# HKUST-Aerial-Robotics/VINS-Mobile

Measured on AMD Instinct MI355X. Metric: VIO frames/sec (KLT+window solve), 640x480/150 feats/W=10, higher is better.
Workload: dtype f64 (solve) / u8+i32+f32 (KLT)

## Files before the change

### include/vio_amd.h

```cpp
#ifndef VIO_AMD_H
#define VIO_AMD_H

#include <stddef.h>
#include <stdint.h>

#ifdef __cplusplus
extern "C" {
#endif

#define VIO_ABI_VERSION 1

#define VIO_OK 0
#define VIO_EINVAL (-1)
#define VIO_ENODEV (-2)
#define VIO_ENOMEM (-3)
#define VIO_ECAP (-4)
#define VIO_ESTATE (-5)
#define VIO_ETIMEOUT (-6)

#define VIO_SIZE_POSE 7
#define VIO_SIZE_SPEEDBIAS 9
#define VIO_MAX_PRIOR_BLOCKS 96

typedef struct VioConfig {
// ... 150 lines not shown
                             int32_t cols, int32_t stride, const double *headers,
                             int32_t publish, VioObs *out_obs ,
                             int32_t *n_obs );

int vio_frontend_submit_images(vio_frontend_t *fe, const uint8_t *gray, int32_t rows,
                               int32_t cols, int32_t stride, int32_t publish);
int vio_frontend_submit_images_async(vio_frontend_t *fe, const uint8_t *gray, int32_t rows, int32_t cols, int32_t stride,
                                     int32_t publish);
int vio_frontend_collect(vio_frontend_t *fe, VioObs *out_obs ,
                         int32_t *n_obs );

int vio_host_register(void *ptr, size_t bytes);
int vio_host_unregister(void *ptr);

int vio_frontend_upload_frames(vio_frontend_t *fe, const uint8_t *gray, int32_t n_frames,
                               int32_t rows, int32_t cols, int32_t stride);
int vio_frontend_step_resident(vio_frontend_t *fe, int32_t frame_index, int32_t publish,
                               void *stream);
int vio_frontend_sync(vio_frontend_t *fe);
int vio_frontend_kernel_ms(vio_frontend_t *fe, double *ms_avg, int32_t *launches);

typedef struct vio_preprocess vio_preprocess_t;
int vio_preprocess_create(int32_t max_frames, int32_t rows, int32_t cols, vio_preprocess_t **out);
void vio_preprocess_destroy(vio_preprocess_t *p);
int vio_preprocess_set_clahe(vio_preprocess_t *p, double clip_limit, int32_t tiles_x, int32_t tiles_y);
int vio_preprocess_run(vio_preprocess_t *p, const uint8_t *pixels, int32_t channels, int32_t n_frames, int32_t stride,
                       uint8_t *gray_out, uint8_t *equalized_out);
int vio_preprocess_run_resident(vio_preprocess_t *p, const void *d_pixels, int32_t channels, int32_t n_frames,
                                int32_t stride, void *d_equalized, void *stream);
int vio_preprocess_sync(vio_preprocess_t *p);
int vio_preprocess_kernel_ms(vio_preprocess_t *p, double *ms_avg, int32_t *launches);

int vio_frontend_get_state(vio_frontend_t *fe, int32_t seq, float *cur_pts ,
                           int32_t *ids, int32_t *track_cnt, int32_t cap, int32_t *n);
int vio_frontend_get_pnp_points(vio_frontend_t *fe, int32_t seq, float *forw_pts , int32_t *ids,
                                int32_t cap, int32_t *n);
int vio_frontend_lk_iterations(vio_frontend_t *fe, int32_t enable, uint64_t *iterations, uint64_t *visits, int32_t levels_cap);

int vio_frontend_set_tracks(vio_frontend_t *fe, int32_t seq, int32_t n, const float *pre_pts,
                            const float *cur_pts, const float *forw_pts, const int32_t *ids,
                            const int32_t *track_cnt, const uint8_t *lk_status);
int vio_frontend_update_tracks(vio_frontend_t *fe, int32_t publish);
int vio_frontend_get_tracks(vio_frontend_t *fe, int32_t seq, float *forw_pts, int32_t *ids,
                            int32_t *track_cnt, int32_t cap, int32_t *n);

int vio_klt_track(const VioConfig *cfg, const uint8_t *prev, const uint8_t *next,
                  int32_t rows, int32_t cols, int32_t stride, const float *prev_pts,
                  int32_t n, float *next_pts, uint8_t *status, float *err);
int vio_good_features(const VioConfig *cfg, const uint8_t *img, const uint8_t *mask,
                      int32_t rows, int32_t cols, int32_t stride, int32_t max_corners,
                      float *corners , int32_t *n_corners);
int vio_fundamental_ransac(const VioConfig *cfg, const float *pts1, const float *pts2,
                           int32_t n, uint8_t *inlier_mask);

typedef struct vio_matcher vio_matcher_t;
int vio_matcher_create(vio_matcher_t **out);
void vio_matcher_destroy(vio_matcher_t *m);
int vio_matcher_search_by_des(vio_matcher_t *m, int32_t n_pairs, const int32_t *n_cur,
                              const int32_t *n_old, const uint64_t *cur_desc,
                              const uint64_t *old_desc, int32_t *best_index,
                              int32_t *best_dist);
int vio_loop_find_connection(vio_matcher_t *m, const VioConfig *cfg, int32_t n_cur,
                             const uint64_t *cur_desc, const float *cur_pts ,
                             int32_t n_old, const uint64_t *old_desc,
                             const float *old_pts ,
                             float *matched_old_pts ,
                             float *matched_old_norm ,
                             uint8_t *status , int32_t *n_inliers);

typedef struct vio_vocabulary vio_vocabulary_t;
int vio_vocabulary_create(const void *blob, size_t bytes, vio_vocabulary_t **out);
int vio_vocabulary_load(const char *path, vio_vocabulary_t **out);
void vio_vocabulary_destroy(vio_vocabulary_t *v);
int vio_vocabulary_info(const vio_vocabulary_t *v, int32_t info[6]);
int vio_vocabulary_get_device(const vio_vocabulary_t *v, int32_t *device);
int vio_vocabulary_transform(vio_vocabulary_t *v, int32_t n_keyframes, const int32_t *n_desc, const uint64_t *desc,
                             int32_t *word_id, double *word_weight, int32_t *bow_count, int32_t *bow_word,
                             double *bow_value, int32_t bow_stride);
typedef struct vio_bow_database vio_bow_database_t;
int vio_bow_database_create(vio_vocabulary_t *v, int32_t max_entries, int32_t max_total_words, vio_bow_database_t **out);
void vio_bow_database_destroy(vio_bow_database_t *d);
int vio_bow_database_size(const vio_bow_database_t *d, int32_t *n_entries);
int vio_bow_database_add(vio_bow_database_t *d, int32_t n, const int32_t *word, const double *value, int32_t *entry_id);
int vio_bow_database_query(vio_bow_database_t *d, int32_t n_queries, const int32_t *bow_count, const int32_t *bow_word,
                           const double *bow_value, int32_t bow_stride, const int32_t *max_id, int32_t max_results,
                           int32_t *n_results, int32_t *entry, double *score, int32_t result_stride);

typedef struct VioLoopDetectorParams {
  int32_t use_nss; float alpha; int32_t k;
  int32_t geom_check;
  int32_t di_levels;
  int32_t dislocal, max_db_results; float min_nss_factor;
  int32_t min_matches_per_group, max_intragroup_gap, max_distance_between_groups, max_distance_between_queries;
  int32_t min_Fpoints; double max_neighbor_ratio;
  double f_threshold, f_confidence; int32_t min_inliers;
} VioLoopDetectorParams;
void vio_loop_detector_params_default(VioLoopDetectorParams *p, float frequency);

enum {
  VIO_LOOP_DETECTED = 0, VIO_LOOP_CLOSE_MATCHES_ONLY = 1, VIO_LOOP_NO_DB_RESULTS = 2, VIO_LOOP_LOW_NSS_FACTOR = 3,
  VIO_LOOP_LOW_SCORES = 4, VIO_LOOP_NO_GROUPS = 5, VIO_LOOP_NO_TEMPORAL_CONSISTENCY = 6,
  VIO_LOOP_NO_GEOMETRICAL_CONSISTENCY = 7
};
typedef struct VioLoopDetection {
  int32_t status;
  int32_t query, match;
// ... 292 lines not shown
```

### vins-mobile_amd/csrc/vio_frontend.hip

```cpp
#include <hip/hip_runtime.h>

#include <type_traits>

#include "vio_exact_math.h"

#include <math.h>
#include <stdint.h>
#include <stdio.h>
#include <string.h>

#include <algorithm>
#include <condition_variable>
#include <memory>
#include <mutex>
#include <thread>
#include <vector>

#include "vio_amd.h"
#include "vio_device.h"
#include "vio_pool.h"

namespace {

constexpr int kMaxLevels = 4;
// ... 132 lines not shown
  }
    VIO_DPPS(0x111, 0xf) VIO_DPPS(0x112, 0xf) VIO_DPPS(0x114, 0xf) VIO_DPPS(0x118, 0xf) VIO_DPPS(0x142, 0xa) VIO_DPPS(0x143, 0xc)
#undef VIO_DPPS
    sp = (float)__builtin_amdgcn_readlane(u[0], 63), sq = (float)__builtin_amdgcn_readlane(u[1], 63);
    return;
  }
  int a = p & 0xffff, b = q & 0xffff, c = p >> 16, d = q >> 16;
#define VIO_DPP4(ctrl, rmask)                                              \
  {                                                                        \
    const int ta = __builtin_amdgcn_update_dpp(0, a, ctrl, rmask, 0xf, false); \
    const int tb = __builtin_amdgcn_update_dpp(0, b, ctrl, rmask, 0xf, false); \
    const int tc = __builtin_amdgcn_update_dpp(0, c, ctrl, rmask, 0xf, false); \
    const int td = __builtin_amdgcn_update_dpp(0, d, ctrl, rmask, 0xf, false); \
    a += ta, b += tb, c += tc, d += td;                                    \
  }
  VIO_DPP4(0x111, 0xf) VIO_DPP4(0x112, 0xf) VIO_DPP4(0x114, 0xf) VIO_DPP4(0x118, 0xf) VIO_DPP4(0x142, 0xa) VIO_DPP4(0x143, 0xc)
#undef VIO_DPP4
  const int sa = __builtin_amdgcn_readlane(a, 63), sb = __builtin_amdgcn_readlane(b, 63), sc = __builtin_amdgcn_readlane(c, 63),
            sd = __builtin_amdgcn_readlane(d, 63);
  sp = (float)sc * 65536.f + (float)sa, sq = (float)sd * 65536.f + (float)sb;
}

__device__ __forceinline__ void wave_sum_exact3(int p, int q, int r, float &sp, float &sq, float &sr) {
  if (wave_all_small(p, q, r)) {
    int w[3] = {p, q, r};
#define VIO_DPPS3(ctrl, rmask)                                                                                       \
  {                                                                                                                   \
    int t[3];                                                                                                         \
    _Pragma("unroll") for (int k = 0; k < 3; k++) t[k] = __builtin_amdgcn_update_dpp(0, w[k], ctrl, rmask, 0xf, false); \
    _Pragma("unroll") for (int k = 0; k < 3; k++) w[k] += t[k];                                                       \
  }
    VIO_DPPS3(0x111, 0xf) VIO_DPPS3(0x112, 0xf) VIO_DPPS3(0x114, 0xf) VIO_DPPS3(0x118, 0xf) VIO_DPPS3(0x142, 0xa) VIO_DPPS3(0x143, 0xc)
#undef VIO_DPPS3
    sp = (float)__builtin_amdgcn_readlane(w[0], 63), sq = (float)__builtin_amdgcn_readlane(w[1], 63), sr = (float)__builtin_amdgcn_readlane(w[2], 63);
    return;
  }
  int u[3] = {p, q, r};
#define VIO_DPPN(N, arr, ctrl, rmask)                                               \
  {                                                                                 \
    int t[N];                                                                       \
    _Pragma("unroll") for (int k = 0; k < N; k++) t[k] = __builtin_amdgcn_update_dpp(0, arr[k], ctrl, rmask, 0xf, false); \
    _Pragma("unroll") for (int k = 0; k < N; k++) arr[k] += t[k];                   \
  }
  VIO_DPPN(3, u, 0x111, 0xf) VIO_DPPN(3, u, 0x112, 0xf) VIO_DPPN(3, u, 0x114, 0xf) VIO_DPPN(3, u, 0x118, 0xf)
  int v[6] = {u[0] & 0xffff, u[1] & 0xffff, u[2] & 0xffff, u[0] >> 16, u[1] >> 16, u[2] >> 16};
  VIO_DPPN(6, v, 0x142, 0xa) VIO_DPPN(6, v, 0x143, 0xc)
#undef VIO_DPPN
  int s[6];
#pragma unroll
  for (int k = 0; k < 6; k++) s[k] = __builtin_amdgcn_readlane(v[k], 63);
  sp = (float)s[3] * 65536.f + (float)s[0], sq = (float)s[4] * 65536.f + (float)s[1], sr = (float)s[5] * 65536.f + (float)s[2];
}

template <bool STATS = false>
__global__ __launch_bounds__(256, 6) void lk_track_kernel(const uint8_t *prev_pyr, const uint8_t *next_pyr, LkParams P,
                                                       const int *n_pts, const float *prev_pts, float *next_pts,
                                                       uint8_t *status, float *err, unsigned long long *stats) {
  __shared__ LkWaveLds lds_all[4];
  const int seq = blockIdx.y;
  const int wave = threadIdx.x >> 6, lane = threadIdx.x & 63;
  const int pt = blockIdx.x * (blockDim.x >> 6) + wave;
  if (pt >= n_pts[seq]) return;
  LkWaveLds &L = lds_all[wave];
  const uint8_t *pp = prev_pyr + (size_t)seq * P.ld.pyr_bytes, *np = next_pyr + (size_t)seq * P.ld.pyr_bytes;
  const size_t pidx = ((size_t)seq * P.cap + pt) * 2;
  const float ptx = prev_pts[pidx], pty = prev_pts[pidx + 1];
  const float half = (kWin - 1) * 0.5f;
  const float FLT_SCALE = 1.f / (1 << 20);
  constexpr int NPX = (kWin * kWin + 63) / 64;
  const int wy0 = min(lane / kWin, 2), wx0 = lane % kWin;
  const int joff = wy0 * kJS + wx0;
  bool st = true;
  float er = 0.f;
  float nxx = 0.f, nxy = 0.f;
  const int max_level = P.ld.levels - 1;
  for (int level = max_level; level >= 0; level--) {
    const int rows = P.ld.rows[level], cols = P.ld.cols[level];
    const uint8_t *I = pp + P.ld.off[level], *J = np + P.ld.off[level];
    if (level == 0) {
      if (P.prev0) I = P.prev0 + (size_t)seq * P.stride0;
      if (P.next0) J = P.next0 + (size_t)seq * P.stride0;
    }
    const float scale = __int_as_float((127 - level) << 23);
    float px = ptx * scale, py = pty * scale;
    float qx, qy;
    if (level == max_level) qx = px, qy = py;
    else qx = nxx * 2.f, qy = nxy * 2.f;
    nxx = qx, nxy = qy;
    px -= half, py -= half;
    int ipx = (int)floorf(px), ipy = (int)floorf(py);
    if (ipx < -kWin || ipx >= cols || ipy < -kWin || ipy >= rows) {
      if (level == 0) st = false, er = 0.f;
      continue;
    }
    float a = px - ipx, b = py - ipy;
    int iw00, iw01, iw10, iw11;
    lk_weights(a, b, iw00, iw01, iw10, iw11);
    wave_lds_fence();
    if (ipx >= 1 && ipx + kIP - 1 <= cols && ipy >= 1 && ipy + kIP - 1 <= rows) {
      const int r = lane / 6, d = lane - 6 * r;
      constexpr int TI = (kIP + 9) / 10;
      uint32_t curs[TI];
#pragma unroll
      for (int t = 0; t < TI; t++) {
        const int ly = r + 10 * t;
        curs[t] = lk_load4(I + (unsigned)(__mul24(ipy - 1 + (ly < kIP ? ly : 0), cols) + ipx - 1 + 4 * d));
      }
// ... 168 lines not shown
      __builtin_memcpy(&bot, &b32, 4);
      return __builtin_amdgcn_sdot2(bot, wbot, (int)__builtin_amdgcn_udot2(top, wtop, (unsigned)Ic[q], false), false) >> (kWBits - 5);
    };
    int nit = 0;
    for (int j = 0; j < P.max_count; j++) {
      int iqx = (int)floorf(qx), iqy = (int)floorf(qy);
      if (iqx < -kWin || iqx >= cols || iqy < -kWin || iqy >= rows) {
        if (level == 0) st = false;
        break;
      }
      if (STATS) nit++;
      if (!j_staged || iqx < jox || iqx > jox + 2 * kJMargin || iqy < joy || iqy > joy + 2 * kJMargin) stage_j(iqx, iqy);
      a = qx - iqx, b = qy - iqy;
      lk_weights(a, b, iw00, iw01, iw10, iw11);
      int pb1 = 0, pb2 = 0;
      const lk_us2 wtop = {(unsigned short)iw00, (unsigned short)iw01};
      const lk_s2 wbot = {(short)iw10, (short)iw11};
      const int jbase = __mul24(iqy - joy, kJS) + (iqx - jox);
#pragma unroll
      for (int h = 0; h < NPP; h++) {
        const int d0 = diff_j(jbase, 2 * h, wtop, wbot), d1 = 2 * h + 1 < NPX ? diff_j(jbase, 2 * h + 1, wtop, wbot) : 0;
        const unsigned pk = __builtin_amdgcn_perm((unsigned)d1, (unsigned)d0, 0x05040100u);
        lk_s2 dp;
        __builtin_memcpy(&dp, &pk, 4);
        pb1 = __builtin_amdgcn_sdot2(dp, IxP[h], pb1, false), pb2 = __builtin_amdgcn_sdot2(dp, IyP[h], pb2, false);
      }
      float fb1, fb2;
      wave_sum_exact2(pb1, pb2, fb1, fb2);
      float b1 = fb1 * FLT_SCALE, b2 = fb2 * FLT_SCALE;
      float ddx = (A12 * b2 - A22 * b1) * D, ddy = (A12 * b1 - A11 * b2) * D;
      qx += ddx, qy += ddy;
      nxx = qx + half, nxy = qy + half;
      if (!(ddx * ddx + ddy * ddy > P.epsilon_sq_f) && (double)ddx * ddx + (double)ddy * ddy <= P.epsilon_sq) break;
      constexpr float kCentiUp = 0.010000000707805157f;
      static_assert((double)kCentiUp > 0.01 && (double)0.01f < 0.01, "float neighbours of 0.01");
      if (j > 0 && fabsf(ddx + pdx) < kCentiUp && fabsf(ddy + pdy) < kCentiUp) {
        nxx -= ddx * 0.5f, nxy -= ddy * 0.5f;
        break;
      }
      pdx = ddx, pdy = ddy;
    }
    if (STATS && lane == 0) {
      unsigned long long *sl = stats + ((blockIdx.x + 7 * blockIdx.y) & 63) * 16;
      atomicAdd(sl + level, (unsigned long long)nit);
      atomicAdd(sl + P.ld.levels + level, 1ull);
    }
    if (st && level == 0) {
      float ex = nxx - half, ey = nxy - half;
      int iex = (int)floorf(ex), iey = (int)floorf(ey);
      if (iex < -kWin || iex >= cols || iey < -kWin || iey >= rows) {
        st = false;
        continue;
      }
      if (!j_staged || iex < jox || iex > jox + 2 * kJMargin || iey < joy || iey > joy + 2 * kJMargin) stage_j(iex, iey);
      float aa = ex - iex, bb = ey - iey;
      lk_weights(aa, bb, iw00, iw01, iw10, iw11);
      int pe = 0;
      const lk_us2 wtop = {(unsigned short)iw00, (unsigned short)iw01};
      const lk_s2 wbot = {(short)iw10, (short)iw11};
      const int jbase = __mul24(iey - joy, kJS) + (iex - jox);
#pragma unroll
      for (int q = 0; q < NPX; q++) {
        const int d = abs(diff_j(jbase, q, wtop, wbot));
        pe += lane < 3 * kWin ? d : 0;
      }
      const int se = wave_sum_i32(pe);
      er = (float)se * 1.f / (32 * kWin * kWin);
    }
  }
  if (lane == 0) {
    next_pts[pidx] = nxx, next_pts[pidx + 1] = nxy;
    status[(size_t)seq * P.cap + pt] = st ? 1 : 0;
    err[(size_t)seq * P.cap + pt] = er;
  }
}

__device__ __attribute__((noinline)) double exact_fn(int which, double x) {
  return which == 0 ? vio_xm::acos_cr(x) : which == 1 ? vio_xm::cos_cr(x) : vio_xm::pow_cr(x, 0.333333333333);
}
__device__ int solve_cubic_dev(const double c[4], double r[3], bool exact) {
  double a0 = c[0], a1 = c[1], a2 = c[2], a3 = c[3];
  double x0 = 0, x1 = 0, x2 = 0;
  int n = 0;
  if (a0 == 0) {
    if (a1 == 0) {
      if (a2 == 0) n = a3 == 0 ? -1 : 0;
      else x0 = -a3 / a2, n = 1;
    } else {
      double d = a2 * a2 - 4 * a1 * a3;
      if (d >= 0) {
        d = sqrt(d);
        double q1 = (-a2 + d) * 0.5, q2 = (a2 + d) * -0.5;
        if (fabs(q1) > fabs(q2)) x0 = q1 / a1, x1 = a3 / q1;
        else x0 = q2 / a1, x1 = a3 / q2;
        n = d > 0 ? 2 : 1;
      }
    }
  } else {
    a0 = 1. / a0, a1 *= a0, a2 *= a0, a3 *= a0;
    double Q = (a1 * a1 - 3 * a2) * (1. / 9), R = (2 * a1 * a1 * a1 - 9 * a1 * a2 + 27 * a3) * (1. / 54);
    double Qcubed = Q * Q * Q, d = Qcubed - R * R;
    const double kPi = 3.14159265358979323846;
    if (d >= 0) {
      const double av = R / sqrt(Qcubed);
      double theta = exact ? exact_fn(0, av) : acos(av), sqrtQ = sqrt(Q);
      double t0 = -2 * sqrtQ, t1 = theta * (1. / 3), t2 = a1 * (1. / 3);
      const double g0 = t1, g1 = t1 + (2. * kPi / 3), g2 = t1 + (4. * kPi / 3);
      if (exact) x0 = t0 * exact_fn(1, g0) - t2, x1 = t0 * exact_fn(1, g1) - t2, x2 = t0 * exact_fn(1, g2) - t2;
      else x0 = t0 * cos(g0) - t2, x1 = t0 * cos(g1) - t2, x2 = t0 * cos(g2) - t2;
      n = 3;
    } else {
      d = sqrt(-d);
      double e = exact ? exact_fn(2, d + fabs(R)) : pow(d + fabs(R), 0.333333333333);
      if (R > 0) e = -e;
      x0 = (e + Q / e) - a1 * (1. / 3);
      n = 1;
    }
  }
  r[0] = x0, r[1] = x1, r[2] = x2;
  return n;
}

struct SevenPointWork {
  double a[63], f1[9], f2[9];
  int colperm[10];
};
// ... 244 lines not shown
    RS_STAMP(0);
    for (int it = tid; it < nb * 7; it += nt) {
      const int h = it / 7, i = it - 7 * h;
      const float4 q = pts(S.idx[h][i]);
      S.ms1[h][2 * i] = q.x, S.ms1[h][2 * i + 1] = q.y;
      S.ms2[h][2 * i] = q.z, S.ms2[h][2 * i + 1] = q.w;
    }
    __syncthreads();
    if (tid < nb) S.coll[tid] = (have_collinear_dev(S.ms1[tid], 7) || have_collinear_dev(S.ms2[tid], 7)) ? 1 : 0;
    __syncthreads();
    if (tid == 0) {
      int first = -1;
      for (int h = 0; h < nb && first < 0; h++)
        if (S.coll[h]) first = h;
      if (first >= 0) {
        unsigned long long st = S.rng_before[first];
        for (int h = first; h < nb; h++) {
          S.valid[h] = draw(st, h, true);
          if (!S.valid[h]) {
            for (int hh = h + 1; hh < nb; hh++) S.valid[hh] = 0;
            break;
          }
        }
        S.rng_state = st;
      }
    }
    __syncthreads();
    RS_STAMP(1);
    for (int h = tid >> 4; h < nb; h += nt >> 4) {
      int n = 0;
      if (S.valid[h]) n = run7point_group(S.ms1[h], S.ms2[h], S.F[h], S.work[h], tid & 15, lmeds);
      if ((tid & 15) == 0) {
        S.nmodels[h] = n < 0 ? 0 : n;
        S.good[h][0] = S.good[h][1] = S.good[h][2] = 0;
      }
    }
    __syncthreads();
    RS_STAMP(2);
    if (lmeds) {
      for (int hk = tid; hk < nb * 3; hk += nt) {
        const int h = hk / 3, k = hk - 3 * h;
        if (k >= S.nmodels[h]) continue;
        int bits[14];
        for (int i = 0; i < count; i++) {
          const float4 q = pts(i);
          const int b = __float_as_int(epipolar_error(S.F[h] + 9 * k, q.x, q.y, q.z, q.w));
          int j = i;
          for (; j > 0 && bits[j - 1] > b; j--) bits[j] = bits[j - 1];
          bits[j] = b;
        }
        S.med[h][k] = (count & 1) ? (double)__int_as_float(bits[count / 2])
                                  : (double)(__int_as_float(bits[count / 2 - 1]) + __int_as_float(bits[count / 2])) * 0.5;
      }
    } else
    for (int item = tid; item < nb * 3 * count; item += nt) {
      int hk = item / count, i = item - hk * count;
      int h = hk / 3, k = hk - 3 * h;
      if (k < S.nmodels[h]) {
        const float4 q = pts(i);
        if (epipolar_inlier(S.F[h] + 9 * k, q.x, q.y, q.z, q.w, t)) atomicAdd(&S.good[h][k], 1);
      }
    }
    __syncthreads();
    RS_STAMP(3);
    if (tid == 0) {
      for (int h = 0; h < nb; h++) {
        if (S.iter >= S.niters) { S.done = 1; break; }
        if (!S.valid[h]) {
          if (S.iter == 0) S.failed_first = 1;
          S.done = 1;
          break;
        }
        for (int k = 0; k < S.nmodels[h]; k++) {
          if (lmeds) {
            if (S.med[h][k] < S.min_median) {
              S.min_median = S.med[h][k];
              for (int q = 0; q < 9; q++) S.bestF[q] = S.F[h][9 * k + q];
            }
            continue;
          }
          int good = S.good[h][k];
          if (good > max(S.max_good, model_points - 1)) {
            S.max_good = good;
            for (int q = 0; q < 9; q++) S.bestF[q] = S.F[h][9 * k + q];
            S.best_h = h;
            S.niters = ransac_update_iters(confidence, (double)(count - good) / count, model_points, S.niters);
          }
        }
        S.iter++;
      }
      if (S.iter >= S.niters) S.done = 1;
    }
    __syncthreads();
    RS_STAMP(4);
    if (prof && tid == 0) prof[6] += 1;
    if (S.done) break;
  }
  if (lmeds && S.min_median < 1.7976931348623157e308 && !S.failed_first) {
    double sigma = 2.5 * 1.4826 * (1 + 5. / (count - model_points)) * sqrt(S.min_median);
    sigma = fmax(sigma, 0.001);
    const float ts = (float)(sigma * sigma);
    for (int i = tid; i < count; i += nt) {
      const float4 q = pts(i);
      mask[i] = epipolar_inlier(S.bestF, q.x, q.y, q.z, q.w, ts) ? 1 : 0;
    }
  } else if (!lmeds && S.max_good > 0 && !S.failed_first) {
    for (int i = tid; i < count; i += nt) {
      const float4 q = pts(i);
      mask[i] = epipolar_inlier(S.bestF, q.x, q.y, q.z, q.w, t) ? 1 : 0;
    }
  } else {
    for (int i = tid; i < count; i += nt) mask[i] = 1;
  }
// ... 74 lines not shown
template <int CAP>
__global__ __launch_bounds__(256, 2) void track_update_kernel(TrackerArrays A, int publish) {
  extern __shared__ __attribute__((aligned(16))) unsigned char smem_raw[];
  TrackShared<CAP> &T = *reinterpret_cast<TrackShared<CAP> *>(smem_raw);
  RansacShared &R = *reinterpret_cast<RansacShared *>(smem_raw + ((sizeof(TrackShared<CAP>) + 15) & ~(size_t)15));
  const int seq = blockIdx.x, tid = threadIdx.x, nt = blockDim.x;
  const size_t base = (size_t)seq * A.cap;
  const int n0 = A.n_pts[seq];
#define TU_STAMP(k)                                                  \
  do {                                                               \
    if (A.prof && seq == 0 && tid == 0) A.prof[k] = clock64();       \
  } while (0)
  TU_STAMP(0);
  if (tid == 0) T.n = n0;
  for (int i = tid; i < n0; i += nt) {
    T.pre[i][0] = A.pre_pts[(base + i) * 2], T.pre[i][1] = A.pre_pts[(base + i) * 2 + 1];
    T.cur[i][0] = A.cur_pts[(base + i) * 2], T.cur[i][1] = A.cur_pts[(base + i) * 2 + 1];
    T.forw[i][0] = A.forw_pts[(base + i) * 2], T.forw[i][1] = A.forw_pts[(base + i) * 2 + 1];
    T.ids[i] = A.ids[base + i], T.cnt[i] = A.track_cnt[base + i];
    int ix = __float2int_rn(T.forw[i][0]), iy = __float2int_rn(T.forw[i][1]);
    bool inb = 1 <= ix && ix < A.cols - 1 && 1 <= iy && iy < A.rows - 1;
    T.keep[i] = (A.lk_status[base + i] && inb) ? 1 : 0;
  }
  __syncthreads();
  TU_STAMP(1);
  shorten_list<CAP, true>(T);
  TU_STAMP(2);
  const int npass = publish ? 2 : 1;
#pragma nounroll
  for (int pass = 0; pass < npass; pass++) {
    if (pass) TU_STAMP(5);
    const int np = T.n;
    if (np >= 8) {
      const float(*from)[2] = pass ? T.pre : T.cur;
      for (int i = tid; i < np; i += nt) {
        const int o = T.idx[i];
        T.pack[i] = make_float4(from[o][0], from[o][1], T.forw[o][0], T.forw[o][1]);
      }
      __syncthreads();
      fundamental_ransac_block(R, PackedPts{T.pack}, np, A.f_thresh, A.f_conf, T.keep, A.prof && seq == 0 ? A.prof + 16 + 8 * pass : nullptr);
      TU_STAMP(pass ? 6 : 3);
      shorten_list<CAP, false>(T);
    }
    if (pass == 0) {
      TU_STAMP(4);
      for (int i = tid; i < T.n; i += nt) {
        const int o = T.idx[i];
        A.pnp_pts[(base + i) * 2] = T.forw[o][0], A.pnp_pts[(base + i) * 2 + 1] = T.forw[o][1];
        A.pnp_ids[base + i] = T.ids[o];
      }
      if (tid == 0) A.n_pnp[seq] = T.n;
    }
  }
  const int n = T.n;
  if (publish) {
    TU_STAMP(7);
    for (int i = tid; i < n; i += nt) {
      const int o = T.idx[i];
      T.ncnt[i] = T.cnt[o] + 1;
      T.ixy[i][0] = __float2int_rn(T.forw[o][0]), T.ixy[i][1] = __float2int_rn(T.forw[o][1]);
    }
    __syncthreads();
    for (int i = tid; i < n; i += nt) {
      int rank = 0, ci = T.ncnt[i];
      for (int j = 0; j < n; j++) rank += (T.ncnt[j] > ci || (T.ncnt[j] == ci && j < i)) ? 1 : 0;
      T.order[rank] = i;
    }
    const int words = (n + 63) / 64;
    __syncthreads();
    TU_STAMP(8);
    for (int q = tid; q < 2 * A.radius + 1; q += nt) T.hw[q] = A.hw[q];
    __syncthreads();
    {
      const int wave = tid >> 6, lane = tid & 63, nwv = nt >> 6;
      constexpr int kW = CAP / 64;
      int jx[kW], jy[kW];
#pragma unroll
      for (int w = 0; w < kW; w++) {
        const int j = min(64 * w + lane, n - 1);
        jx[w] = T.ixy[j][0], jy[w] = T.ixy[j][1];
      }
      const int rad = A.radius;
      for (int i = wave; i < n; i += nwv) {
        const int ix = T.ixy[i][0], iy = T.ixy[i][1];
#pragma unroll
        for (int w = 0; w < kW; w++) {
          if (w < words) {
            const int dy = iy - jy[w], dx = ix - jx[w];
            const int h = T.hw[rad + min(max(dy, -rad), rad)];
            const bool in = 64 * w + lane < n && dy >= -rad && dy <= rad && dx >= -h && dx <= h;
            const unsigned long long bits = __builtin_amdgcn_ballot_w64(in);
            if (lane == 0) T.inside[i][w] = bits;
          }
        }
      }
    }
    __syncthreads();
    TU_STAMP(9);
    if (tid < 64) {
      const int lane = tid;
      unsigned long long mine = 0;
      int c = 0;
      for (int r0 = 0; r0 < n; r0 += 64) {
        const int my_i = r0 + lane < n ? T.order[r0 + lane] : 0;
        const int cnt = n - r0 < 64 ? n - r0 : 64;
        unsigned long long kept = 0;
        for (int q0 = 0; q0 < cnt; q0 += 8) {
          int is[8];
          unsigned long long rows[8];
#pragma unroll
          for (int u = 0; u < 8; u++) {
            is[u] = __builtin_amdgcn_readlane(my_i, (q0 + u) & 63);
            rows[u] = lane < words ? T.inside[is[u]][lane] : 0ull;
          }
#pragma unroll
          for (int u = 0; u < 8; u++) {
            const int i = is[u];
            const bool keep_it = q0 + u < cnt && __builtin_amdgcn_ballot_w64((rows[u] & mine) != 0) == 0;
            const unsigned long long bit = keep_it ? 1ULL << (i & 63) : 0ull;
            mine |= lane == (i >> 6) ? bit : 0ull;
            kept |= (unsigned long long)keep_it << ((q0 + u) & 63);
          }
        }
        if (lane < cnt) {
          const bool k = (kept >> lane) & 1ull;
          T.keep[my_i] = k ? 1 : 0;
          if (k) T.pos[my_i] = c + __builtin_popcountll(kept & ((1ull << lane) - 1ull));
        }
        c += __builtin_popcountll(kept);
      }
      if (lane == 0) T.n = c;
    }
    __syncthreads();
    TU_STAMP(10);
    for (int i = tid; i < n; i += nt)
      if (T.keep[i]) {
        const int p = T.pos[i], o = T.idx[i];
        A.forw_pts[(base + p) * 2] = T.forw[o][0], A.forw_pts[(base + p) * 2 + 1] = T.forw[o][1];
        A.ids[base + p] = T.ids[o], A.track_cnt[base + p] = T.ncnt[i];
        A.kept_xy[(base + p) * 2] = T.ixy[i][0], A.kept_xy[(base + p) * 2 + 1] = T.ixy[i][1];
      }
    if (tid == 0) A.n_kept[seq] = T.n, A.n_forw[seq] = T.n;
  } else {
    for (int i = tid; i < n; i += nt) {
      const int o = T.idx[i];
      A.forw_pts[(base + i) * 2] = T.forw[o][0], A.forw_pts[(base + i) * 2 + 1] = T.forw[o][1];
// ... 655 lines not shown
}

int fe_step(vio_frontend *fe, const uint8_t *d_frames , int publish, hipStream_t st, bool keep_frames = false) {
  const int S = fe->n_seq, rows = fe->cfg.image_rows, cols = fe->cfg.image_cols, cap = fe->cap;
  const size_t img_bytes = (size_t)rows * cols;
  const int fidx = fe->have_img ? 1 - fe->cur_idx : fe->cur_idx;
  uint8_t *forw = fe->pyr[fidx].p;
  const bool fused0 = fe->ld.levels >= 2 && cols % 4 == 0 && fe->ld.cols[1] % 4 == 0 && cols >= 8 && fe->ld.pyr_bytes % 4 == 0 &&
                      img_bytes % 4 == 0 && (uintptr_t)d_frames % 4 == 0 && (uintptr_t)forw % 4 == 0 && fe->ld.off[1] % 4 == 0;
  const bool alias0 = keep_frames && fused0 && !vio::env_flag("VIO_AMD_COPY_LEVEL0");
  fe->lvl0[fidx] = alias0 ? d_frames : nullptr;
  if (!fused0) {
    const int vec_ok = img_bytes % 16 == 0 && fe->ld.pyr_bytes % 16 == 0 && (uintptr_t)d_frames % 16 == 0 &&
                       (uintptr_t)forw % 16 == 0;
    dim3 grd((unsigned)((img_bytes + 16 * 256 - 1) / (16 * 256)), S);
    hipLaunchKernelGGL(copy_frames_kernel, grd, dim3(256), 0, st, d_frames, img_bytes, forw, fe->ld.pyr_bytes, img_bytes,
                       vec_ok);
  }
  for (int l = 1; l < fe->ld.levels; l++) {
    const uint8_t *sp = forw + fe->ld.off[l - 1];
    uint8_t *dp = forw + fe->ld.off[l];
    const int sc = fe->ld.cols[l - 1], dc = fe->ld.cols[l];
    if (l == 1 && fused0) {
      dim3 blk(256), grd((dc + kPdW - 1) / kPdW, (fe->ld.rows[1] + kPd4H * kPd4T - 1) / (kPd4H * kPd4T), S);
      if (alias0)
        hipLaunchKernelGGL(pyr_down4_kernel<false>, grd, blk, 0, st, d_frames, img_bytes, dp, fe->ld.pyr_bytes, rows, cols, fe->ld.rows[1], dc,
                           (uint8_t *)nullptr);
      else
        hipLaunchKernelGGL(pyr_down4_kernel<true>, grd, blk, 0, st, d_frames, img_bytes, dp, fe->ld.pyr_bytes, rows, cols, fe->ld.rows[1], dc, forw);
      continue;
    }
    const bool dwords = sc % 4 == 0 && dc % 4 == 0 && sc >= 8 && fe->ld.pyr_bytes % 4 == 0 && (uintptr_t)sp % 4 == 0 && (uintptr_t)dp % 4 == 0;
    if (dwords) {
      dim3 blk(256), grd((dc + kPdW - 1) / kPdW, (fe->ld.rows[l] + kPd4H * kPd4T - 1) / (kPd4H * kPd4T), S);
      hipLaunchKernelGGL(pyr_down4_kernel<false>, grd, blk, 0, st, sp, fe->ld.pyr_bytes, dp, fe->ld.pyr_bytes, fe->ld.rows[l - 1], sc, fe->ld.rows[l], dc,
                         (uint8_t *)nullptr);
    } else {
      dim3 blk(256), grd((dc + kPdW - 1) / kPdW, (fe->ld.rows[l] + kPdH - 1) / kPdH, S);
      hipLaunchKernelGGL(pyr_down_kernel, grd, blk, 0, st, sp, dp, fe->ld.pyr_bytes, fe->ld.rows[l - 1], sc, fe->ld.rows[l], dc);
    }
  }
  if (!fe->have_img) {
    fe->have_img = true;
    fe->cur_idx = fidx;
  } else {
    LkParams P;
    P.ld = fe->ld, P.cap = cap;
    P.max_count = std::min(std::max(fe->cfg.lk_max_iters, 0), 100);
    double eps = std::min(std::max(fe->cfg.lk_eps, 0.), 10.);
    P.epsilon_sq = eps * eps, P.epsilon_sq_f = lk_eps_screen(eps * eps), P.min_eig = (float)fe->cfg.lk_min_eig;
    P.prev0 = fe->lvl0[fe->cur_idx], P.next0 = fe->lvl0[fidx], P.stride0 = img_bytes;
    dim3 grd((cap + 3) / 4, S);
    if (fe->lk_stats_on && fe->lk_stats.p)
      hipLaunchKernelGGL((lk_track_kernel<true>), grd, dim3(256), 0, st, fe->pyr[fe->cur_idx].p, forw, P, fe->n_pts.p, fe->cur_pts.p,
                         fe->forw_pts.p, fe->lk_status.p, fe->lk_err.p, fe->lk_stats.p);
    else
      hipLaunchKernelGGL((lk_track_kernel<false>), grd, dim3(256), 0, st, fe->pyr[fe->cur_idx].p, forw, P, fe->n_pts.p, fe->cur_pts.p,
                         fe->forw_pts.p, fe->lk_status.p, fe->lk_err.p, (unsigned long long *)nullptr);
  }
  int rcu = launch_track_update(fe, publish, st);
  if (rcu != VIO_OK) return rcu;
  if (publish) {
    dim3 tb(256), tg((cols + kDetWaves * kDetW - 1) / (kDetWaves * kDetW), fe->nseg, S);
    hipLaunchKernelGGL(detect_kernel<false>, tg, tb, 0, st, alias0 ? d_frames : forw, alias0 ? img_bytes : fe->ld.pyr_bytes, (const uint8_t *)nullptr, (size_t)0,
                       fe->kept_xy.p, fe->n_kept.p, cap, fe->hw.p, fe->cfg.min_dist, fe->max_bits.p, rows, cols, fe->cand.p,
                       fe->seg_cap, fe->n_cand.p, fe->detect_always ? (const int *)nullptr : fe->n_forw.p, fe->cfg.max_corners);
    SelectParams SP;
    SP.cap = cap, SP.rows = rows, SP.cols = cols, SP.max_corners = fe->cfg.max_corners, SP.min_dist = (float)fe->cfg.min_dist;
    SP.fx = fe->cfg.fx, SP.fy = fe->cfg.fy, SP.cx = fe->cfg.cx, SP.cy = fe->cfg.cy;
    hipLaunchKernelGGL(corner_select_kernel, dim3(S), dim3(kSelThreads), 0, st, fe->cand.p, fe->seg_cap, fe->nseg, fe->n_cand.p,
                       fe->max_bits.p, fe->cfg.quality_level, SP, fe->forw_pts.p, fe->cur_pts.p, fe->pre_pts.p, fe->ids.p,
                       fe->track_cnt.p, fe->n_forw.p, fe->n_pts.p, fe->n_id.p, fe->obs.p, fe->n_obs.p, fe->cs_prof ? fe->d_cs_prof.p : nullptr);
    if (fe->cs_prof) {
      long long h[5];
      if (hipStreamSynchronize(st) == hipSuccess && hipMemcpy(h, fe->d_cs_prof.p, sizeof(h), hipMemcpyDeviceToHost) == hipSuccess)
        fprintf(stderr, "corner_select cycles (sequence 0): threshold %lld, selection %lld, ids %lld, outputs %lld, total %lld\n", h[1] - h[0],
                h[2] - h[1], h[3] - h[2], h[4] - h[3], h[4] - h[0]);
    }
  }
  HIP_OK(hipGetLastError());
  fe->cur_idx = fidx;
  return VIO_OK;
}

}

extern "C" {

int vio_frontend_create(const VioConfig *cfg, int32_t n_seq, vio_frontend_t **out) {
  if (!cfg || !out || n_seq < 1) return VIO_EINVAL;
  if (cfg->lk_win != kWin || cfg->lk_levels < 0 || cfg->lk_levels >= kMaxLevels || cfg->max_corners < 1 ||
      cfg->max_corners > kMaxCap || cfg->image_rows < 32 || cfg->image_cols < 32 || cfg->min_dist < 0 || cfg->min_dist > kMaxRadius ||
      cfg->image_rows > 32767 || cfg->image_cols > 65535)
    return VIO_EINVAL;
  if (!vio::device_ready("the front-end")) return VIO_ENODEV;
  vio_frontend *fe = new vio_frontend();
  fe->device = vio::current_device();
  fe->cfg = *cfg, fe->n_seq = n_seq, fe->cap = cfg->max_corners;
  fe->detect_always = vio::env_flag("VIO_AMD_DETECT_ALWAYS");
  fe->cs_prof = vio::env_flag("VIO_AMD_CS_PROF") && fe->d_cs_prof.ensure(8) == VIO_OK;
  LevelDims &ld = fe->ld;
  ld.rows[0] = cfg->image_rows, ld.cols[0] = cfg->image_cols, ld.off[0] = 0, ld.levels = 1;
  size_t off = (size_t)ld.rows[0] * ld.cols[0];
  for (int l = 1; l <= cfg->lk_levels; l++) {
    int r = (ld.rows[l - 1] + 1) / 2, c = (ld.cols[l - 1] + 1) / 2;
    if (c <= kWin || r <= kWin) break;
    ld.rows[l] = r, ld.cols[l] = c, ld.off[l] = off, off += (size_t)r * c, ld.levels = l + 1;
  }
  ld.pyr_bytes = (off + 255) & ~(size_t)255;
  const size_t S = n_seq, cap = fe->cap;
  fe->nseg = (cfg->image_rows + kDetR - 1) / kDetR;
// ... 363 lines not shown
                            int32_t *n) {
  if (!fe || seq < 0 || seq >= fe->n_seq || !n) return VIO_EINVAL;
  if (fe->pending) return VIO_ESTATE;
  VIO_ON_DEVICE_OF(fe);
  HIP_OK(hipDeviceSynchronize());
  int m = 0;
  HIP_OK(hipMemcpy(&m, fe->n_forw.p + seq, sizeof(int), hipMemcpyDeviceToHost));
  *n = m;
  if (m > cap) return VIO_ECAP;
  const size_t base = (size_t)seq * fe->cap;
  if (m > 0) {
    HIP_OK(hipMemcpy(forw_pts, fe->forw_pts.p + base * 2, sizeof(float) * 2 * m, hipMemcpyDeviceToHost));
    HIP_OK(hipMemcpy(ids, fe->ids.p + base, sizeof(int) * m, hipMemcpyDeviceToHost));
    HIP_OK(hipMemcpy(track_cnt, fe->track_cnt.p + base, sizeof(int) * m, hipMemcpyDeviceToHost));
  }
  return VIO_OK;
}

using FrontendPtr = std::unique_ptr<vio_frontend, void (*)(vio_frontend_t *)>;

int vio_klt_track(const VioConfig *cfg, const uint8_t *prev, const uint8_t *next, int32_t rows, int32_t cols, int32_t stride,
                  const float *prev_pts, int32_t n, float *next_pts, uint8_t *status, float *err) {
  if (!cfg || !prev || !next || n < 0 || (n > 0 && (!prev_pts || !next_pts || !status || !err))) return VIO_EINVAL;
  if (n == 0) return VIO_OK;
  VioConfig c = *cfg;
  c.image_rows = rows, c.image_cols = cols, c.max_corners = std::min(std::max(n, 1), kMaxCap);
  if (n > kMaxCap) return VIO_ECAP;
  vio_frontend *raw = nullptr;
  int rc = vio_frontend_create(&c, 1, &raw);
  if (rc != VIO_OK) return rc;
  const FrontendPtr fe(raw, vio_frontend_destroy);
  const size_t px = (size_t)rows * cols;
  DevBuf<uint8_t> d;
  if (d.ensure(2 * px) != VIO_OK) return VIO_ENOMEM;
  if (hipMemcpy2D(d.p, cols, prev, stride, cols, rows, hipMemcpyHostToDevice) != hipSuccess) return VIO_ENODEV;
  if (hipMemcpy2D(d.p + px, cols, next, stride, cols, rows, hipMemcpyHostToDevice) != hipSuccess) return VIO_ENODEV;
  hipStream_t st = fe->stream;
  for (int k = 0; k < 2; k++) {
    uint8_t *dst = fe->pyr[k].p;
    if (hipMemcpyAsync(dst, d.p + k * px, px, hipMemcpyDeviceToDevice, st) != hipSuccess) return VIO_ENODEV;
    for (int l = 1; l < fe->ld.levels; l++) {
      dim3 blk(256), grd((fe->ld.cols[l] + kPdW - 1) / kPdW, (fe->ld.rows[l] + kPdH - 1) / kPdH, 1);
      hipLaunchKernelGGL(pyr_down_kernel, grd, blk, 0, st, dst + fe->ld.off[l - 1], dst + fe->ld.off[l], fe->ld.pyr_bytes,
                         fe->ld.rows[l - 1], fe->ld.cols[l - 1], fe->ld.rows[l], fe->ld.cols[l]);
    }
  }
  if (hipMemcpyAsync(fe->cur_pts.p, prev_pts, sizeof(float) * 2 * n, hipMemcpyHostToDevice, st) != hipSuccess) return VIO_ENODEV;
  if (hipMemcpyAsync(fe->n_pts.p, &n, sizeof(int), hipMemcpyHostToDevice, st) != hipSuccess) return VIO_ENODEV;
  LkParams P;
  P.ld = fe->ld, P.cap = fe->cap, P.max_count = std::min(std::max(c.lk_max_iters, 0), 100);
  double eps = std::min(std::max(c.lk_eps, 0.), 10.);
  P.epsilon_sq = eps * eps, P.epsilon_sq_f = lk_eps_screen(eps * eps), P.min_eig = (float)c.lk_min_eig;
  P.prev0 = P.next0 = nullptr, P.stride0 = 0;
  hipLaunchKernelGGL((lk_track_kernel<false>), dim3((fe->cap + 3) / 4, 1), dim3(256), 0, st, fe->pyr[0].p, fe->pyr[1].p, P, fe->n_pts.p,
                     fe->cur_pts.p, fe->forw_pts.p, fe->lk_status.p, fe->lk_err.p, (unsigned long long *)nullptr);
  if (hipStreamSynchronize(st) != hipSuccess || hipGetLastError() != hipSuccess) return VIO_ENODEV;
  if (hipMemcpy(next_pts, fe->forw_pts.p, sizeof(float) * 2 * n, hipMemcpyDeviceToHost) != hipSuccess) return VIO_ENODEV;
  if (hipMemcpy(status, fe->lk_status.p, n, hipMemcpyDeviceToHost) != hipSuccess) return VIO_ENODEV;
  if (hipMemcpy(err, fe->lk_err.p, sizeof(float) * n, hipMemcpyDeviceToHost) != hipSuccess) return VIO_ENODEV;
  return VIO_OK;
}

int vio_good_features(const VioConfig *cfg, const uint8_t *img, const uint8_t *mask, int32_t rows, int32_t cols, int32_t stride,
                      int32_t max_corners, float *corners, int32_t *n_corners) {
  if (!cfg || !img || !corners || !n_corners || max_corners < 1) return VIO_EINVAL;
  if (max_corners > kMaxCap) return VIO_ECAP;
  VioConfig c = *cfg;
  c.image_rows = rows, c.image_cols = cols, c.max_corners = max_corners;
  vio_frontend *raw = nullptr;
  int rc = vio_frontend_create(&c, 1, &raw);
  if (rc != VIO_OK) return rc;
  const FrontendPtr fe(raw, vio_frontend_destroy);
  const size_t px = (size_t)rows * cols;
  hipStream_t st = fe->stream;
  if (hipMemcpy2D(fe->pyr[0].p, cols, img, stride, cols, rows, hipMemcpyHostToDevice) != hipSuccess) return VIO_ENODEV;
  if (fe->mask.ensure(px) != VIO_OK) return VIO_ENOMEM;
  if (mask) {
    if (hipMemcpy2D(fe->mask.p, cols, mask, stride, cols, rows, hipMemcpyHostToDevice) != hipSuccess) return VIO_ENODEV;
  } else if (hipMemset(fe->mask.p, 255, px) != hipSuccess) {
    return VIO_ENODEV;
  }
  if (hipMemset(fe->max_bits.p, 0, sizeof(unsigned) * fe->nseg) != hipSuccess ||
      hipMemset(fe->n_cand.p, 0, sizeof(int) * fe->nseg) != hipSuccess)
    return VIO_ENODEV;
  dim3 tb(256), tg((cols + kDetWaves * kDetW - 1) / (kDetWaves * kDetW), fe->nseg, 1);
  hipLaunchKernelGGL(detect_kernel<true>, tg, tb, 0, st, fe->pyr[0].p, fe->ld.pyr_bytes, fe->mask.p, px, fe->kept_xy.p, fe->n_kept.p,
                     fe->cap, fe->hw.p, c.min_dist, fe->max_bits.p, rows, cols, fe->cand.p, fe->seg_cap, fe->n_cand.p, (const int *)nullptr, 0);
  SelectParams SP;
  SP.cap = fe->cap, SP.rows = rows, SP.cols = cols, SP.max_corners = max_corners, SP.min_dist = (float)c.min_dist;
  SP.fx = c.fx, SP.fy = c.fy, SP.cx = c.cx, SP.cy = c.cy;
  hipLaunchKernelGGL(corner_select_kernel, dim3(1), dim3(kSelThreads), 0, st, fe->cand.p, fe->seg_cap, fe->nseg, fe->n_cand.p, fe->max_bits.p,
                     c.quality_level, SP, fe->forw_pts.p, fe->cur_pts.p, fe->pre_pts.p, fe->ids.p, fe->track_cnt.p, fe->n_forw.p, fe->n_pts.p,
                     fe->n_id.p, fe->obs.p, fe->n_obs.p, (long long *)nullptr);
  if (hipStreamSynchronize(st) != hipSuccess || hipGetLastError() != hipSuccess) return VIO_ENODEV;
  int n = 0;
  if (hipMemcpy(&n, fe->n_pts.p, sizeof(int), hipMemcpyDeviceToHost) != hipSuccess) return VIO_ENODEV;
  *n_corners = n;
  if (n > 0 && hipMemcpy(corners, fe->forw_pts.p, sizeof(float) * 2 * n, hipMemcpyDeviceToHost) != hipSuccess) return VIO_ENODEV;
  return VIO_OK;
}

__global__ __launch_bounds__(256) void ransac_only_kernel(const float *p1, const float *p2, int n, float thresh, double conf,
                                                          uint8_t *mask) {
  extern __shared__ __attribute__((aligned(16))) unsigned char smem_raw[];
  RansacShared &R = *reinterpret_cast<RansacShared *>(smem_raw);
  fundamental_ransac_block(R, GlobalPts{p1, p2}, n, thresh, conf, mask);
}

int vio_fundamental_ransac(const VioConfig *cfg, const float *pts1, const float *pts2, int32_t n, uint8_t *inlier_mask) {
  if (!cfg || !pts1 || !pts2 || !inlier_mask || n < 0) return VIO_EINVAL;
  if (n == 0) return VIO_OK;
  int ndev = 0;
  if (hipGetDeviceCount(&ndev) != hipSuccess || ndev < 1) return VIO_ENODEV;
  DevBuf<float> d1, d2;
  DevBuf<uint8_t> dm;
  if (d1.ensure((size_t)2 * n) != VIO_OK || d2.ensure((size_t)2 * n) != VIO_OK || dm.ensure((size_t)n) != VIO_OK) return VIO_ENOMEM;
  if (hipMemcpy(d1.p, pts1, sizeof(float) * 2 * n, hipMemcpyHostToDevice) != hipSuccess) return VIO_ENODEV;
  if (hipMemcpy(d2.p, pts2, sizeof(float) * 2 * n, hipMemcpyHostToDevice) != hipSuccess) return VIO_ENODEV;
  hipLaunchKernelGGL(ransac_only_kernel, dim3(1), dim3(256), sizeof(RansacShared), 0, d1.p, d2.p, n, (float)cfg->f_threshold,
                     cfg->f_confidence, dm.p);
  if (hipDeviceSynchronize() != hipSuccess || hipGetLastError() != hipSuccess) return VIO_ENODEV;
  if (hipMemcpy(inlier_mask, dm.p, n, hipMemcpyDeviceToHost) != hipSuccess) return VIO_ENODEV;
  return VIO_OK;
}

}

__global__ __launch_bounds__(256) void ransac_batch_kernel(const float *p1, const float *p2, const int *count, int stride, int min_count,
                                                           float thresh, double conf, uint8_t *mask) {
  extern __shared__ __attribute__((aligned(16))) unsigned char smem_raw[];
  RansacShared &R = *reinterpret_cast<RansacShared *>(smem_raw);
  const int p = blockIdx.x, n = count[p];
  if (n < min_count || n > stride) return;
  fundamental_ransac_block(R, GlobalPts{p1 + 2 * (size_t)p * stride, p2 + 2 * (size_t)p * stride}, n, thresh, conf, mask + (size_t)p * stride);
}

namespace vio {
int fundamental_ransac_batch(hipStream_t st, const float *p1, const float *p2, const int *count, int n_prob, int stride, int min_count,
                             float thresh, double conf, uint8_t *mask) {
  if (n_prob < 1) return VIO_OK;
  hipLaunchKernelGGL(ransac_batch_kernel, dim3(n_prob), dim3(256), sizeof(RansacShared), st, p1, p2, count, stride, min_count, thresh, conf,
                     mask);
  HIP_OK(hipGetLastError());
  return VIO_OK;
}
}
```

### vins-mobile_amd/frontend.py

```python
import ctypes as C

import numpy as np

from . import abi

_u8p, _fp, _ip = C.POINTER(C.c_uint8), C.POINTER(C.c_float), C.POINTER(C.c_int32)


_OBS_DTYPE = np.dtype({"names": ["id", "x", "y", "z"], "formats": ["<i4", "<f8", "<f8", "<f8"],
                       "offsets": [0, 8, 16, 24], "itemsize": 32})
assert C.sizeof(abi.VioObs) == 32


class FeatureTracker:
    def __init__(self, cfg=None, n_seq=1):
        self.lib = abi.load_product()
        self.cfg = cfg if cfg is not None else abi.default_config()
        self.n_seq = n_seq
        self._h = C.c_void_p()
        rc = self.lib.vio_frontend_create(C.byref(self.cfg), n_seq, C.byref(self._h))
        if rc != abi.VIO_OK:
            raise RuntimeError("vio_frontend_create failed rc=%d (a gfx950 device is required)" % rc)
        self._frames = None

# ... 102 lines not shown
        self._check(self.lib.vio_frontend_step_resident(self._h, frame_index, 1 if publish else 0,
                                                        C.c_void_p(stream) if stream else None), "step_resident")

    def sync(self):
        self._check(self.lib.vio_frontend_sync(self._h), "sync")

    def kernel_ms(self):
        ms = C.c_double()
        n = C.c_int32()
        self._check(self.lib.vio_frontend_kernel_ms(self._h, C.byref(ms), C.byref(n)), "kernel_ms")
        return ms.value, n.value


def klt_track(cfg, prev, nxt, pts):
    lib = abi.load_product()
    prev, nxt = np.ascontiguousarray(prev, np.uint8), np.ascontiguousarray(nxt, np.uint8)
    pts = np.ascontiguousarray(pts, np.float32).reshape(-1, 2)
    n = len(pts)
    out = np.zeros((n, 2), np.float32)
    st = np.zeros(n, np.uint8)
    err = np.zeros(n, np.float32)
    rc = lib.vio_klt_track(C.byref(cfg), prev.ctypes.data_as(_u8p), nxt.ctypes.data_as(_u8p), prev.shape[0], prev.shape[1],
                           prev.shape[1], pts.ctypes.data_as(_fp), n, out.ctypes.data_as(_fp), st.ctypes.data_as(_u8p),
                           err.ctypes.data_as(_fp))
    if rc != abi.VIO_OK:
        raise RuntimeError("vio_klt_track rc=%d" % rc)
    return out, st, err


def good_features(cfg, img, mask, max_corners):
    lib = abi.load_product()
    img = np.ascontiguousarray(img, np.uint8)
    corners = np.zeros((max_corners, 2), np.float32)
    n = C.c_int32()
    mp = np.ascontiguousarray(mask, np.uint8).ctypes.data_as(_u8p) if mask is not None else None
    rc = lib.vio_good_features(C.byref(cfg), img.ctypes.data_as(_u8p), mp, img.shape[0], img.shape[1], img.shape[1],
                               max_corners, corners.ctypes.data_as(_fp), C.byref(n))
    if rc != abi.VIO_OK:
        raise RuntimeError("vio_good_features rc=%d" % rc)
    return corners[: n.value].copy()


def fundamental_ransac(cfg, p1, p2):
    lib = abi.load_product()
    p1 = np.ascontiguousarray(p1, np.float32).reshape(-1, 2)
    p2 = np.ascontiguousarray(p2, np.float32).reshape(-1, 2)
    m = np.zeros(len(p1), np.uint8)
    rc = lib.vio_fundamental_ransac(C.byref(cfg), p1.ctypes.data_as(_fp), p2.ctypes.data_as(_fp), len(p1), m.ctypes.data_as(_u8p))
    if rc != abi.VIO_OK:
        raise RuntimeError("vio_fundamental_ransac rc=%d" % rc)
    return m


class Preprocessor:

    def __init__(self, rows, cols, max_frames=1, lib=None):
        self.lib = lib or abi.load_product()
        self.rows, self.cols, self.max_frames = rows, cols, max_frames
        self._h = C.c_void_p()
        rc = self.lib.vio_preprocess_create(max_frames, rows, cols, C.byref(self._h))
        if rc != 0:
            raise RuntimeError("vio_preprocess_create failed: %d" % rc)

    def close(self):
        if self._h:
            self.lib.vio_preprocess_destroy(self._h)
            self._h = C.c_void_p()

    def set_clahe(self, clip_limit=3.0, tiles_x=8, tiles_y=8):
        rc = self.lib.vio_preprocess_set_clahe(self._h, float(clip_limit), tiles_x, tiles_y)
        if rc != 0:
            raise RuntimeError("vio_preprocess_set_clahe failed: %d" % rc)

    def run(self, frames):
        frames = np.ascontiguousarray(frames, np.uint8)
        ch = 4 if frames.ndim == 4 else 1
        n = frames.shape[0]
        assert frames.shape[1:3] == (self.rows, self.cols)
        gray, eq = np.zeros((n, self.rows, self.cols), np.uint8), np.zeros((n, self.rows, self.cols), np.uint8)
        u8p = C.POINTER(C.c_uint8)
        rc = self.lib.vio_preprocess_run(self._h, frames.ctypes.data_as(u8p), ch, n, self.cols * ch, gray.ctypes.data_as(u8p),
                                         eq.ctypes.data_as(u8p))
        if rc != 0:
            raise RuntimeError("vio_preprocess_run failed: %d" % rc)
        return gray, eq

    def run_resident(self, d_pixels, channels, n_frames, d_equalized, stream=None):
        rc = self.lib.vio_preprocess_run_resident(self._h, C.c_void_p(d_pixels), channels, n_frames, self.cols * channels,
                                                  C.c_void_p(d_equalized), C.c_void_p(stream or 0))
        if rc != 0:
            raise RuntimeError("vio_preprocess_run_resident failed: %d" % rc)

    def sync(self):
        rc = self.lib.vio_preprocess_sync(self._h)
        if rc != 0:
            raise RuntimeError("vio_preprocess_sync failed: %d" % rc)

    def kernel_ms(self):
        ms, n = C.c_double(), C.c_int32()
        self.lib.vio_preprocess_kernel_ms(self._h, C.byref(ms), C.byref(n))
        return ms.value, n.value
```

Baseline: 186,000.

## Skip unused LK error in frontend, wave-per-model RANSAC scoring, batch neighbor masks

The frontend LK kernel now gets a template flag that skips the final-level error computation and its store, because the pipeline never reads the error. The one-off API keeps computing it. RANSAC hypothesis scoring changes from per-item atomics to whole waves that each score one model with ballot/popcount. The track-update neighbor-mask loop processes several points per iteration and does a single lane-indexed store, and a batched RANSAC host API is added. These cut atomic contention, LDS traffic and wasted error work, at the cost of more registers and a change to the behavior of the err output.

```diff
diff --git a/include/vio_amd.h b/include/vio_amd.h
--- a/include/vio_amd.h
+++ b/include/vio_amd.h
@@ -226,6 +226,9 @@
                       float *corners , int32_t *n_corners);
 int vio_fundamental_ransac(const VioConfig *cfg, const float *pts1, const float *pts2,
                            int32_t n, uint8_t *inlier_mask);
+int vio_fundamental_ransac_batch(const VioConfig *cfg, const float *pts1, const float *pts2,
+                                 const int32_t *counts, int32_t n_prob, int32_t stride,
+                                 int32_t min_count, uint8_t *inlier_masks);
 
 typedef struct vio_matcher vio_matcher_t;
 int vio_matcher_create(vio_matcher_t **out);
diff --git a/vins-mobile_amd/csrc/vio_frontend.hip b/vins-mobile_amd/csrc/vio_frontend.hip
--- a/vins-mobile_amd/csrc/vio_frontend.hip
+++ b/vins-mobile_amd/csrc/vio_frontend.hip
@@ -208,7 +208,7 @@
   sp = (float)s[3] * 65536.f + (float)s[0], sq = (float)s[4] * 65536.f + (float)s[1], sr = (float)s[5] * 65536.f + (float)s[2];
 }
 
-template <bool STATS = false>
+template <bool STATS = false, bool ERR = true>
 __global__ __launch_bounds__(256, 6) void lk_track_kernel(const uint8_t *prev_pyr, const uint8_t *next_pyr, LkParams P,
                                                        const int *n_pts, const float *prev_pts, float *next_pts,
                                                        uint8_t *status, float *err, unsigned long long *stats) {
@@ -483,6 +483,7 @@
         st = false;
         continue;
       }
+      if (!ERR) continue;
       if (!j_staged || iex < jox || iex > jox + 2 * kJMargin || iey < joy || iey > joy + 2 * kJMargin) stage_j(iex, iey);
       float aa = ex - iex, bb = ey - iey;
       lk_weights(aa, bb, iw00, iw01, iw10, iw11);
@@ -502,7 +503,7 @@
   if (lane == 0) {
     next_pts[pidx] = nxx, next_pts[pidx + 1] = nxy;
     status[(size_t)seq * P.cap + pt] = st ? 1 : 0;
-    err[(size_t)seq * P.cap + pt] = er;
+    if (ERR) err[(size_t)seq * P.cap + pt] = er;
   }
 }
 
@@ -853,13 +854,25 @@
         S.med[h][k] = (count & 1) ? (double)__int_as_float(bits[count / 2])
                                   : (double)(__int_as_float(bits[count / 2 - 1]) + __int_as_float(bits[count / 2])) * 0.5;
       }
-    } else
-    for (int item = tid; item < nb * 3 * count; item += nt) {
-      int hk = item / count, i = item - hk * count;
-      int h = hk / 3, k = hk - 3 * h;
-      if (k < S.nmodels[h]) {
-        const float4 q = pts(i);
-        if (epipolar_inlier(S.F[h] + 9 * k, q.x, q.y, q.z, q.w, t)) atomicAdd(&S.good[h][k], 1);
+    } else {
+      const int lane = tid & 63, wave = __builtin_amdgcn_readfirstlane(tid >> 6), nwv = nt >> 6;
+      const int nm = lane < nb ? S.nmodels[lane] : 0;
+      unsigned long long live = __builtin_amdgcn_ballot_w64(nm > 0) | __builtin_amdgcn_ballot_w64(nm > 1) << 16 |
+                                __builtin_amdgcn_ballot_w64(nm > 2) << 32;
+      for (int turn = 0; live; live &= live - 1, turn = turn + 1 == nwv ? 0 : turn + 1) {
+        if (turn != wave) continue;
+        const int bit = __builtin_ctzll(live), k = bit >> 4, h = bit & 15;
+        double F[9];
+#pragma unroll
+        for (int q = 0; q < 9; q++) F[q] = S.F[h][9 * k + q];
+        int good = 0;
+        const int cnt = __builtin_amdgcn_readfirstlane(count);
+        for (int i0 = 0; i0 < cnt; i0 += 64) {
+          const int i = i0 + lane;
+          const float4 q = pts(i < cnt ? i : cnt - 1);
+          good += __builtin_popcountll(__builtin_amdgcn_ballot_w64(i < cnt && epipolar_inlier(F, q.x, q.y, q.z, q.w, t)));
+        }
+        if (lane == 0) S.good[h][k] = good;
       }
     }
     __syncthreads();
@@ -1040,7 +1053,7 @@
       if (tid == 0) A.n_pnp[seq] = T.n;
     }
   }
-  const int n = T.n;
+  const int n = __builtin_amdgcn_readfirstlane(T.n);
   if (publish) {
     TU_STAMP(7);
     for (int i = tid; i < n; i += nt) {
@@ -1069,17 +1082,30 @@
         jx[w] = T.ixy[j][0], jy[w] = T.ixy[j][1];
       }
       const int rad = A.radius;
-      for (int i = wave; i < n; i += nwv) {
-        const int ix = T.ixy[i][0], iy = T.ixy[i][1];
-#pragma unroll
-        for (int w = 0; w < kW; w++) {
-          if (w < words) {
-            const int dy = iy - jy[w], dx = ix - jx[w];
-            const int h = T.hw[rad + min(max(dy, -rad), rad)];
+      constexpr int kIB = kW <= 4 ? 8 : 4;
+      for (int i0 = wave * kIB; i0 < n; i0 += nwv * kIB) {
+        int ix[kIB], iy[kIB];
+#pragma unroll
+        for (int u = 0; u < kIB; u++) {
+          const int i = min(i0 + u, n - 1);
+          ix[u] = T.ixy[i][0], iy[u] = T.ixy[i][1];
+        }
+        int hh[kIB][kW];
+#pragma unroll
+        for (int u = 0; u < kIB; u++)
+#pragma unroll
+          for (int w = 0; w < kW; w++) hh[u][w] = T.hw[rad + min(max(iy[u] - jy[w], -rad), rad)];
+#pragma unroll
+        for (int u = 0; u < kIB; u++) {
+          unsigned long long row = 0;
+#pragma unroll
+          for (int w = 0; w < kW; w++) {
+            const int dy = iy[u] - jy[w], dx = ix[u] - jx[w], h = hh[u][w];
             const bool in = 64 * w + lane < n && dy >= -rad && dy <= rad && dx >= -h && dx <= h;
             const unsigned long long bits = __builtin_amdgcn_ballot_w64(in);
-            if (lane == 0) T.inside[i][w] = bits;
+            row = lane == w ? bits : row;
           }
+          if (lane < words && i0 + u < n) T.inside[i0 + u][lane] = row;
         }
       }
     }
@@ -1841,11 +1867,11 @@
     P.prev0 = fe->lvl0[fe->cur_idx], P.next0 = fe->lvl0[fidx], P.stride0 = img_bytes;
     dim3 grd((cap + 3) / 4, S);
     if (fe->lk_stats_on && fe->lk_stats.p)
-      hipLaunchKernelGGL((lk_track_kernel<true>), grd, dim3(256), 0, st, fe->pyr[fe->cur_idx].p, forw, P, fe->n_pts.p, fe->cur_pts.p,
-                         fe->forw_pts.p, fe->lk_status.p, fe->lk_err.p, fe->lk_stats.p);
+      hipLaunchKernelGGL((lk_track_kernel<true, false>), grd, dim3(256), 0, st, fe->pyr[fe->cur_idx].p, forw, P, fe->n_pts.p, fe->cur_pts.p,
+                         fe->forw_pts.p, fe->lk_status.p, (float *)nullptr, fe->lk_stats.p);
     else
-      hipLaunchKernelGGL((lk_track_kernel<false>), grd, dim3(256), 0, st, fe->pyr[fe->cur_idx].p, forw, P, fe->n_pts.p, fe->cur_pts.p,
-                         fe->forw_pts.p, fe->lk_status.p, fe->lk_err.p, (unsigned long long *)nullptr);
+      hipLaunchKernelGGL((lk_track_kernel<false, false>), grd, dim3(256), 0, st, fe->pyr[fe->cur_idx].p, forw, P, fe->n_pts.p, fe->cur_pts.p,
+                         fe->forw_pts.p, fe->lk_status.p, (float *)nullptr, (unsigned long long *)nullptr);
   }
   int rcu = launch_track_update(fe, publish, st);
   if (rcu != VIO_OK) return rcu;
@@ -2315,7 +2341,7 @@
   double eps = std::min(std::max(c.lk_eps, 0.), 10.);
   P.epsilon_sq = eps * eps, P.epsilon_sq_f = lk_eps_screen(eps * eps), P.min_eig = (float)c.lk_min_eig;
   P.prev0 = P.next0 = nullptr, P.stride0 = 0;
-  hipLaunchKernelGGL((lk_track_kernel<false>), dim3((fe->cap + 3) / 4, 1), dim3(256), 0, st, fe->pyr[0].p, fe->pyr[1].p, P, fe->n_pts.p,
+  hipLaunchKernelGGL((lk_track_kernel<false, true>), dim3((fe->cap + 3) / 4, 1), dim3(256), 0, st, fe->pyr[0].p, fe->pyr[1].p, P, fe->n_pts.p,
                      fe->cur_pts.p, fe->forw_pts.p, fe->lk_status.p, fe->lk_err.p, (unsigned long long *)nullptr);
   if (hipStreamSynchronize(st) != hipSuccess || hipGetLastError() != hipSuccess) return VIO_ENODEV;
   if (hipMemcpy(next_pts, fe->forw_pts.p, sizeof(float) * 2 * n, hipMemcpyDeviceToHost) != hipSuccess) return VIO_ENODEV;
@@ -2408,3 +2434,25 @@
   return VIO_OK;
 }
 }
+
+extern "C" int vio_fundamental_ransac_batch(const VioConfig *cfg, const float *pts1, const float *pts2, const int32_t *counts, int32_t n_prob,
+                                            int32_t stride, int32_t min_count, uint8_t *inlier_masks) {
+  if (!cfg || !pts1 || !pts2 || !counts || !inlier_masks || n_prob < 0 || stride < 1 || min_count < 8) return VIO_EINVAL;
+  if (n_prob == 0) return VIO_OK;
+  int ndev = 0;
+  if (hipGetDeviceCount(&ndev) != hipSuccess || ndev < 1) return VIO_ENODEV;
+  const size_t np = (size_t)n_prob * stride;
+  DevBuf<float> d1, d2;
+  DevBuf<int> dc;
+  DevBuf<uint8_t> dm;
+  if (d1.ensure(2 * np) != VIO_OK || d2.ensure(2 * np) != VIO_OK || dc.ensure((size_t)n_prob) != VIO_OK || dm.ensure(np) != VIO_OK) return VIO_ENOMEM;
+  if (hipMemcpy(d1.p, pts1, sizeof(float) * 2 * np, hipMemcpyHostToDevice) != hipSuccess) return VIO_ENODEV;
+  if (hipMemcpy(d2.p, pts2, sizeof(float) * 2 * np, hipMemcpyHostToDevice) != hipSuccess) return VIO_ENODEV;
+  if (hipMemcpy(dc.p, counts, sizeof(int) * n_prob, hipMemcpyHostToDevice) != hipSuccess) return VIO_ENODEV;
+  if (hipMemcpy(dm.p, inlier_masks, np, hipMemcpyHostToDevice) != hipSuccess) return VIO_ENODEV;
+  const int rc = vio::fundamental_ransac_batch(0, d1.p, d2.p, dc.p, n_prob, stride, min_count, (float)cfg->f_threshold, cfg->f_confidence, dm.p);
+  if (rc != VIO_OK) return rc;
+  if (hipDeviceSynchronize() != hipSuccess || hipGetLastError() != hipSuccess) return VIO_ENODEV;
+  if (hipMemcpy(inlier_masks, dm.p, np, hipMemcpyDeviceToHost) != hipSuccess) return VIO_ENODEV;
+  return VIO_OK;
+}
diff --git a/vins-mobile_amd/frontend.py b/vins-mobile_amd/frontend.py
--- a/vins-mobile_amd/frontend.py
+++ b/vins-mobile_amd/frontend.py
@@ -178,6 +178,22 @@
     return m
 
 
+def fundamental_ransac_batch(cfg, p1, p2, counts, min_count, fill=7):
+    lib = abi.load_product()
+    p1, p2 = np.ascontiguousarray(p1, np.float32), np.ascontiguousarray(p2, np.float32)
+    counts = np.ascontiguousarray(counts, np.int32)
+    n_prob, stride = p1.shape[0], p1.shape[1]
+    assert p1.shape == p2.shape == (n_prob, stride, 2) and len(counts) == n_prob
+    m = np.full((n_prob, stride), fill, np.uint8)
+    lib.vio_fundamental_ransac_batch.argtypes = [C.POINTER(abi.VioConfig), _fp, _fp, C.POINTER(C.c_int32), C.c_int32, C.c_int32,
+                                                 C.c_int32, _u8p]
+    rc = lib.vio_fundamental_ransac_batch(C.byref(cfg), p1.ctypes.data_as(_fp), p2.ctypes.data_as(_fp),
+                                          counts.ctypes.data_as(C.POINTER(C.c_int32)), n_prob, stride, min_count, m.ctypes.data_as(_u8p))
+    if rc != abi.VIO_OK:
+        raise RuntimeError("vio_fundamental_ransac_batch rc=%d" % rc)
+    return m
+
+
 class Preprocessor:
 
     def __init__(self, rows, cols, max_frames=1, lib=None):
```

New measurement: 187,600 (median of 6 runs). No clear change (+0.8%).
